# HueCodes/sudoku-vision

Hardware: AMD Instinct MI355X
Metric: end-to-end frames/sec (1080p->81 digits) (higher is better)
Workload: dtype f32

## Files before the change

### include/sudoku_vision_hip.h

```cpp
#ifndef SUDOKU_VISION_HIP_H
#define SUDOKU_VISION_HIP_H

#include <stddef.h>
#include <stdint.h>

#ifdef __cplusplus
extern "C" {
#endif

typedef struct sv_ctx sv_ctx;

typedef enum sv_status {
    SV_OK = 0,
    SV_ERR_BAD_ARG = -1,
    SV_ERR_HIP = -2,
    SV_ERR_NO_WEIGHTS = -3,
    SV_ERR_UNSUPPORTED = -4,
    SV_ERR_DEGENERATE = -5,
    SV_ERR_BUFFER = -6
} sv_status;

#define SV_CNN_PARAMS 421642
#define SV_CELLS 81
#define SV_CELL_PX 784
// ... 23 lines not shown

int sv_conv_kernel_info(sv_ctx *ctx, int *algo, int *mfma_f32_conv2_per_cell, int *mfma_f32_conv1_per_cell,
                        int *mfma_f16_conv_per_cell, int *mfma_f16_fc_per_cell);

int sv_load_weights_f32(sv_ctx *ctx, const float *blob);


int sv_gray_u8(sv_ctx *ctx, const uint8_t *bgr , int n, int H, int W, ptrdiff_t pitch,
               ptrdiff_t img_stride, uint8_t *gray , void *stream);

int sv_blur_u8(sv_ctx *ctx, const uint8_t *src , int n, int H, int W, int ksize,
               uint8_t *dst , void *stream);

int sv_adaptive_threshold_u8(sv_ctx *ctx, const uint8_t *src , int n, int H, int W,
                             int block, double c, int type_inv, uint8_t *dst , void *stream);

int sv_preprocess_u8(sv_ctx *ctx, const uint8_t *bgr , int n, int H, int W, ptrdiff_t pitch,
                     ptrdiff_t img_stride, uint8_t *binary , void *stream);

int sv_preprocess_warp_cells_u8(sv_ctx *ctx, const uint8_t *bgr , int n, int H, int W, ptrdiff_t pitch, ptrdiff_t img_stride,
                                uint8_t *binary , const double *minv , uint8_t *cells , void *stream);

int sv_preprocess_bits_u8(sv_ctx *ctx, const uint8_t *bgr , int n, int H, int W, ptrdiff_t pitch,
                          ptrdiff_t img_stride, uint32_t *bits , void *stream);

int sv_despeckle_bits(sv_ctx *ctx, uint32_t *bits , int n, int H, int W, void *stream);

int sv_despeckle_u8(sv_ctx *ctx, const uint8_t *binary , int n, int H, int W,
                    uint8_t *out , uint32_t *packed , void *stream);

long sv_sparse_bits_record_bytes(int H, int W, long cap_values);
int sv_pack_sparse_bits(sv_ctx *ctx, const uint32_t *bits , int n, int H, int W,
                        uint8_t *records , long record_stride, void *stream);

int sv_copy_to_pinned_host(sv_ctx *ctx, const void *src , void *dst_host , size_t bytes, void *stream);


int sv_find_grid_corners_u8(const uint8_t *binary , int H, int W, ptrdiff_t pitch,
                            double min_area_ratio, double epsilon_ratio, int *corners );

int sv_find_grid_corners_batch_u8(const uint8_t *binary , int n, int H, int W, ptrdiff_t pitch,
                                  ptrdiff_t img_stride, double min_area_ratio, double epsilon_ratio,
                                  int *corners , uint8_t *found , int threads);

int sv_find_grid_corners_bits_batch(const uint32_t *bits , int n, int H, int W,
                                    double min_area_ratio, double epsilon_ratio,
                                    int *corners , uint8_t *found , int threads);

int sv_host_pool_set_affinity(const int *cpus , int n);

int sv_find_grid_corners_sparse_batch(const uint8_t *records , long record_stride, int n, int H, int W,
                                      double min_area_ratio, double epsilon_ratio,
                                      int *corners , uint8_t *found , int threads);

int sv_sparse_bits_expand(const uint8_t *record , int H, int W, uint32_t *bits );

int sv_find_contours_u8(const uint8_t *binary , int H, int W, ptrdiff_t pitch,
                        int *points , long cap_points, int *sizes ,
                        int cap_contours, long *n_points, int *n_contours);

int sv_find_contours_bits(const uint32_t *bits , int H, int W, int *points, long cap_points, int *sizes, int cap_contours,
                          long *n_points, int *n_contours);

int sv_contour_area_i32(const int *xy , int n, double *area);
int sv_arc_length_i32(const int *xy , int n, int closed, double *length);
int sv_approx_poly_dp_i32(const int *xy , int n, double epsilon, int closed,
// ... 157 lines not shown
```

### sudoku-vision_amd/_native.py

```python
import ctypes as C
import os

_HERE = os.path.dirname(os.path.abspath(__file__))
LIB_PATH = os.path.join(_HERE, "csrc", "libsudokuvision_hip.so")
XCHECK_LIB_PATH = os.path.join(_HERE, "csrc", "libsudokuvision_xcheck.so")
ABI_VERSION = 2

SV_OK = 0
ERR_NAMES = {-1: "SV_ERR_BAD_ARG", -2: "SV_ERR_HIP", -3: "SV_ERR_NO_WEIGHTS", -4: "SV_ERR_UNSUPPORTED",
             -5: "SV_ERR_DEGENERATE", -6: "SV_ERR_BUFFER"}

_p, _i, _l, _d, _f, _pd = C.c_void_p, C.c_int, C.c_long, C.c_double, C.c_float, C.c_ssize_t

SIGNATURES = {
    "sv_version": [],
    "sv_last_error": [],
    "sv_ctx_create": [_i, C.POINTER(_p)],
    "sv_ctx_destroy": [_p],
    "sv_ctx_reserve": [_p, _l],
    "sv_ctx_set_precision": [_p, _i],
    "sv_load_weights_f32": [_p, _p],
    "sv_timing_begin": [_p],
    "sv_timing_end": [_p, _p, _p, _i],
    "sv_ctx_set_cnn_kernels": [_p, _i],
    "sv_conv_kernel_info": [_p, _p, _p, _p, _p, _p],
    "sv_gray_u8": [_p, _p, _i, _i, _i, _pd, _pd, _p, _p],
    "sv_blur_u8": [_p, _p, _i, _i, _i, _i, _p, _p],
    "sv_adaptive_threshold_u8": [_p, _p, _i, _i, _i, _i, _d, _i, _p, _p],
    "sv_preprocess_u8": [_p, _p, _i, _i, _i, _pd, _pd, _p, _p],
    "sv_solve_sudoku": [_p, _p, _p],
    "sv_despeckle_u8": [_p, _p, _i, _i, _i, _p, _p, _p],
    "sv_preprocess_bits_u8": [_p, _p, _i, _i, _i, _pd, _pd, _p, _p],
    "sv_preprocess_warp_cells_u8": [_p, _p, _i, _i, _i, _pd, _pd, _p, _p, _p, _p],
    "sv_despeckle_bits": [_p, _p, _i, _i, _i, _p],
    "sv_copy_to_pinned_host": [_p, _p, _p, C.c_size_t, _p],
    "sv_sparse_bits_record_bytes": [_i, _i, _l],
    "sv_pack_sparse_bits": [_p, _p, _i, _i, _i, _p, _l, _p],
    "sv_find_grid_corners_sparse_batch": [_p, _l, _i, _i, _i, _d, _d, _p, _p, _i],
    "sv_sparse_bits_expand": [_p, _i, _i, _p],
    "sv_host_pool_set_affinity": [_p, _i],
    "sv_find_grid_corners_bits_batch": [_p, _i, _i, _i, _d, _d, _p, _p, _i],
    "sv_corners_to_minv": [_p, _i, _i, _f, _p],
    "sv_corners_to_minv_batch": [_p, _i, _i, _f, _p, _p],
    "sv_find_grid_corners_u8": [_p, _i, _i, _pd, _d, _d, _p],
    "sv_find_grid_corners_batch_u8": [_p, _i, _i, _i, _pd, _pd, _d, _d, _p, _p, _i],
    "sv_find_contours_u8": [_p, _i, _i, _pd, _p, _l, _p, _i, _p, _p],
    "sv_find_contours_bits": [_p, _i, _i, _p, _l, _p, _i, _p, _p],
    "sv_contour_area_i32": [_p, _i, _p],
    "sv_arc_length_i32": [_p, _i, _i, _p],
    "sv_approx_poly_dp_i32": [_p, _i, _d, _i, _p, _p],
    "sv_warp_perspective_u8": [_p, _p, _i, _i, _pd, _i, _p, _i, _p, _p],
    "sv_extract_cells_u8": [_p, _p, _i, _i, _pd, _i, _i, _i, _i, _p, _p],
    "sv_warp_cells_u8": [_p, _p, _i, _i, _i, _pd, _pd, _p, _p, _p],
    "sv_resize_linear_u8": [_p, _p, _i, _i, _pd, _p, _i, _i, _p],
    "sv_cell_ink_ratio_u8": [_p, _p, _l, _i, _p, _p, _p],
    "sv_preprocess_cells_u8": [_p, _p, _l, _p, _p],
    "sv_jpeg_parse": [_p, C.c_size_t, _p],
    "sv_jpeg_entropy_decode": [_p, C.c_size_t, _p, _p, _i],
    "sv_jpeg_entropy_decode_sparse": [_p, C.c_size_t, _p, _p, _p, _l, _p, _p, _i],
    "sv_jpeg_entropy_decode_batch": [_p, _p, _i, _p, _p, _p, _p, _p, _p, _p, _i, _p],
    "sv_jpeg_reconstruct_bgr_u8": [_p, _p, _p, _p, _p, _pd, _p],
    "sv_jpeg_reconstruct_sparse_bgr_u8": [_p, _p, _p, _p, _p, _p, _p, _pd, _p],
    "sv_softmax_topk_f32": [_p, _p, _l, _i, _p, _p, _p],
    "sv_cnn_forward_f32": [_p, _p, _l, _p, _p, _p, _p],
    "sv_cnn_forward_cells_u8": [_p, _p, _l, _i, _p, _p, _p, _p],
    "sv_frames_to_digits": [_p, _p, _i, _i, _i, _pd, _pd, _p, _i, _p, _p, _p, _p, _p],
    "sv_load_weights_v3_f32": [_p, _p, _l, _i],
    "sv_cnn3_forward_f32": [_p, _p, _l, _p, _p, _p, _p, _p],
    "sv_cnn3_forward_cells_u8": [_p, _p, _l, _i, _p, _p, _p, _p],
    "sv_frames_to_digits_v3": [_p, _p, _i, _i, _i, _pd, _pd, _p, _i, _p, _p, _p, _p, _p],
# ... 73 lines not shown
```

### sudoku-vision_amd/csrc/k4_despeckle.hip

```cpp
#include "sv_device.h"
#include "sv_internal.h"

namespace {

typedef unsigned long long u64;
typedef unsigned int u32;

__device__ __forceinline__ u64 lane_shift_up(u64 v)
{
    const u32 lo = (u32)__builtin_amdgcn_update_dpp(0, (int)(u32)v, 0x138, 0xf, 0xf, true);
    const u32 hi = (u32)__builtin_amdgcn_update_dpp(0, (int)(u32)(v >> 32), 0x138, 0xf, 0xf, true);
    return ((u64)hi << 32) | lo;
}
__device__ __forceinline__ u64 lane_shift_down(u64 v)
{
    const u32 lo = (u32)__builtin_amdgcn_update_dpp(0, (int)(u32)v, 0x130, 0xf, 0xf, true);
    const u32 hi = (u32)__builtin_amdgcn_update_dpp(0, (int)(u32)(v >> 32), 0x130, 0xf, 0xf, true);
    return ((u64)hi << 32) | lo;
}
__device__ __forceinline__ u64 fill_runs(u64 f, u64 fr, u64 g)
{
    u64 up = ((f + g) ^ f) & f;
    const u64 gr = __brevll(g | up);
    const u64 dn = ((fr + gr) ^ fr) & fr;
// ... 145 lines not shown
        if (ok1[t] && (u32)(keep >> 32) != (u32)(f[t] >> 32)) row[k0[t] + 1] = (u32)(keep >> 32);
    }
}

__global__ __launch_bounds__(512) void k_despeckle_bits_band(u32 *__restrict__ bits, int H, int wpr, int pitch, int ox, int oy, int tiles_x, int tiles_y)
{
    extern __shared__ u32 band[];
    const int lane = threadIdx.x & 63, wave = threadIdx.x >> 6;
    const int ty = blockIdx.x % tiles_y;
    const long frame = blockIdx.x / tiles_y;
    const int y0 = ty * T - oy;
    u32 *img = bits + frame * H * (long)wpr;
    for (int r = wave; r < T; r += 8) {
        const int y = y0 + r;
        const bool ok = y >= 0 && y < H;
        for (int k = lane; k < wpr; k += 64) band[r * pitch + k] = ok ? img[(long)y * wpr + k] : 0u;
    }
    __syncthreads();
    const int y = y0 + lane;
    const bool row_ok = y >= 0 && y < H;
    u32 *row = img + (long)(row_ok ? y : 0) * wpr;
    const u32 *brow = band + lane * pitch;
    for (int tx = wave; tx < tiles_x; tx += 8) {
        const int k0 = (tx * T - ox) >> 5;
        const bool ok0 = k0 >= 0 && k0 < wpr, ok1 = k0 + 1 < wpr;
        const u64 f = (ok0 ? (u64)brow[k0] : 0ull) | (ok1 ? (u64)brow[k0 + 1] << 32 : 0ull);
        const u64 keep = ring_connected(f, lane);
        if (keep == f || !row_ok) continue;
        if (ok0 && (u32)keep != (u32)f) row[k0] = (u32)keep;
        if (ok1 && (u32)(keep >> 32) != (u32)(f >> 32)) row[k0 + 1] = (u32)(keep >> 32);
    }
}

__global__ __launch_bounds__(256) void k_copy_to_host(const uint4 *__restrict__ src, uint4 *__restrict__ dst, size_t n16, const u8 *__restrict__ tail_src,
                                                      u8 *__restrict__ tail_dst, int tail)
{
    for (size_t i = blockIdx.x * (size_t)256 + threadIdx.x; i < n16; i += (size_t)gridDim.x * 256) dst[i] = src[i];
    if (blockIdx.x == 0 && (int)threadIdx.x < tail) tail_dst[threadIdx.x] = tail_src[threadIdx.x];
}

template <bool KEEP>
__global__ __launch_bounds__(1024) void k_pack_sparse(const u32 *__restrict__ bits, int H, int wpr, int gpr, u8 *__restrict__ records, long stride,
                                                      unsigned cap_values)
{
    extern __shared__ u32 cnt[];
    const int tid = threadIdx.x, lane = tid & 63, wave = tid >> 6, G = H * gpr;
    u32 *wsum = cnt + G;
    const u32 *fb = bits + (size_t)blockIdx.x * H * wpr;
    u8 *rec = records + (size_t)blockIdx.x * stride;
    u64 *masks = (u64 *)(rec + 8);
    u32 *values = (u32 *)(rec + 8 + 8 * (size_t)G);
    constexpr int U = 8, TRIPS = 9;
    u32 kept[KEEP ? TRIPS : 1][U];
    auto load_trip = [&](int g0, u32 (&w)[U]) {
#pragma unroll
        for (int u = 0; u < U; u++) {
            const int g = g0 + u, y = g / gpr, k = (g - y * gpr) * 64 + lane;
            w[u] = (g < G && k < wpr) ? fb[(size_t)y * wpr + k] : 0u;
        }
    };
    auto count_trip = [&](int g0, const u32 (&w)[U]) {
#pragma unroll
        for (int u = 0; u < U; u++) {
            const u64 m = __ballot(w[u] != 0);
            if (lane == 0 && g0 + u < G) { masks[g0 + u] = m; cnt[g0 + u] = (u32)__popcll(m); }
        }
// ... 53 lines not shown
}

int svk_despeckle_bits(uint32_t *bits, int n, int H, int W, hipStream_t s)
{
    for (int pass = 0; pass < 2; pass++) {
        const int o = pass ? T / 2 : 0;
        const int tiles_x = (W + o + T - 1) / T, tiles_y = (H + o + T - 1) / T;
        const int wpr = W >> 5, pitch = wpr | 1;
        if ((size_t)T * pitch * 4 <= 65536) {
            hipLaunchKernelGGL(k_despeckle_bits_band, dim3((unsigned)(n * tiles_y)), dim3(512), (size_t)T * pitch * 4, s, bits, H, wpr, pitch, o, o, tiles_x, tiles_y);
            SV_LAUNCH_CHECK("k_despeckle_bits_band");
            continue;
        }
        const long ngroups = (long)n * ((tiles_x + TPW - 1) / TPW) * tiles_y;
        hipLaunchKernelGGL(k_despeckle_bits, dim3((unsigned)((ngroups + 3) / 4)), dim3(256), 0, s, bits, H, wpr, o, o, tiles_x, tiles_y, ngroups);
        SV_LAUNCH_CHECK("k_despeckle_bits");
    }
    return SV_OK;
}

int svk_pack_sparse_bits(const u32 *bits, int n, int H, int W, u8 *records, long stride, hipStream_t s)
{
    const int wpr = W >> 5, gpr = (wpr + 63) / 64, G = H * gpr;
    const long cap = (stride - 8 - 8L * G) / 4;
    const unsigned capu = (unsigned)(cap > 0xffffffffL ? 0xffffffffL : cap);
    if (G <= 16 * 9 * 8)
        hipLaunchKernelGGL(k_pack_sparse<true>, dim3((unsigned)n), dim3(1024), (size_t)(G + 16) * 4, s, bits, H, wpr, gpr, records, stride, capu);
    else
        hipLaunchKernelGGL(k_pack_sparse<false>, dim3((unsigned)n), dim3(1024), (size_t)(G + 16) * 4, s, bits, H, wpr, gpr, records, stride, capu);
    SV_LAUNCH_CHECK("k_pack_sparse");
    return SV_OK;
}

int svk_copy_to_host(const void *src, void *dst_host, size_t bytes, hipStream_t s)
{
    const size_t n16 = bytes / 16;
    const int tail = (int)(bytes - n16 * 16);
    size_t wgs = (n16 + 255) / 256;
    wgs = wgs < 1 ? 1 : (wgs > 64 ? 64 : wgs);
    hipLaunchKernelGGL(k_copy_to_host, dim3((unsigned)wgs), dim3(256), 0, s, (const uint4 *)src, (uint4 *)dst_host, n16, (const u8 *)src + n16 * 16,
                       (u8 *)dst_host + n16 * 16, tail);
    SV_LAUNCH_CHECK("k_copy_to_host");
    return SV_OK;
}

int svk_despeckle(const u8 *src, int n, int H, int W, u8 *dst, u32 *packed, hipStream_t s)
{
    for (int pass = 0; pass < 2; pass++) {
        const int o = pass ? T / 2 : 0;
        const int tiles_x = (W + o + T - 1) / T, tiles_y = (H + o + T - 1) / T;
        const long ntiles = (long)n * tiles_x * tiles_y;
        hipLaunchKernelGGL(k_despeckle, dim3((unsigned)((ntiles + 3) / 4)), dim3(256), 0, s, pass ? dst : src, dst, pass ? packed : (u32 *)nullptr, H, W, o, o,
                           tiles_x, tiles_y, ntiles);
        SV_LAUNCH_CHECK("k_despeckle");
    }
    return SV_OK;
}
```

### sudoku-vision_amd/csrc/sv_api.cpp

```cpp
#include <algorithm>
#include <cmath>
#include <cstdlib>
#include <cstring>
#include <vector>

#include "sv_internal.h"

static thread_local char g_err[512] = "";

int sv_fail(int code, const char *fmt, ...)
{
    va_list ap;
    va_start(ap, fmt);
    vsnprintf(g_err, sizeof g_err, fmt, ap);
    va_end(ap);
    return code;
}

extern "C" const char *sv_last_error(void) { return g_err; }
extern "C" int sv_version(void) { return 2; }

extern "C" int sv_ctx_create(int device, sv_ctx **out)
{
    if (!out) return sv_fail(SV_ERR_BAD_ARG, "sv_ctx_create: out is NULL");
    int count = 0;
    SV_HIP(hipGetDeviceCount(&count));
    if (device < 0 || device >= count) return sv_fail(SV_ERR_BAD_ARG, "sv_ctx_create: device %d of %d", device, count);
    SV_HIP(hipSetDevice(device));
    hipDeviceProp_t prop;
    SV_HIP(hipGetDeviceProperties(&prop, device));
    sv_ctx *c = new sv_ctx();
    c->device = device;
    c->num_cus = prop.multiProcessorCount > 0 ? prop.multiProcessorCount : 256;
    *out = c;
    return SV_OK;
}

template <class W>
static void free_weights(W &w)
{
    for (void *p : w.allocs) (void)hipFree(p);
    w = W();
}

extern "C" int sv_ctx_destroy(sv_ctx *ctx)
{
    if (!ctx) return SV_OK;
    (void)hipSetDevice(ctx->device);
    free_weights(ctx->w);
    free_weights(ctx->w3);
    if (ctx->v3_act) (void)hipFree(ctx->v3_act);
    if (ctx->features) (void)hipFree(ctx->features);
    if (ctx->cells) (void)hipFree(ctx->cells);
    if (ctx->cells2) (void)hipFree(ctx->cells2);
    if (ctx->jpeg_planes) (void)hipFree(ctx->jpeg_planes);
    if (ctx->pp2) (void)hipFree(ctx->pp2);
    if (ctx->k1_list) (void)hipFree(ctx->k1_list);
    if (ctx->range_flag) (void)hipFree(ctx->range_flag);
    for (auto &t : ctx->timeline) { (void)hipEventDestroy(t.t0); (void)hipEventDestroy(t.t1); }
    for (auto &e : ctx->event_pool) (void)hipEventDestroy(e);
    delete ctx;
    return SV_OK;
}

int sv_ensure_scratch(sv_ctx *ctx, long cells)
{
    if (cells <= ctx->cap_cells) return SV_OK;
    SV_HIP(hipSetDevice(ctx->device));
    if (ctx->features) SV_HIP(hipFree(ctx->features));
    if (ctx->cells) SV_HIP(hipFree(ctx->cells));
    if (ctx->cells2) SV_HIP(hipFree(ctx->cells2));
    ctx->features = nullptr;
    ctx->cells = nullptr;
    ctx->cells2 = nullptr;
    ctx->cap_cells = 0;
    SV_HIP(hipMalloc((void **)&ctx->features, sizeof(float) * 3136 * (size_t)cells));
    SV_HIP(hipMalloc((void **)&ctx->cells, (size_t)SV_CELL_PX * (size_t)cells));
    SV_HIP(hipMalloc((void **)&ctx->cells2, (size_t)SV_CELL_PX * (size_t)cells));
    ctx->cap_cells = cells;
    return SV_OK;
}

static int sv_ensure_scratch_v3(sv_ctx *ctx, long cells)
{
    const long want = cells < SV_V3_SUBBATCH ? cells : SV_V3_SUBBATCH;
    if (want <= ctx->cap_v3) return SV_OK;
    SV_HIP(hipSetDevice(ctx->device));
    if (ctx->v3_act) SV_HIP(hipFree(ctx->v3_act));
    ctx->v3_act = nullptr;
// ... 314 lines not shown

extern "C" int sv_despeckle_bits(sv_ctx *ctx, uint32_t *bits, int n, int H, int W, void *stream)
{
    REQUIRE(ctx && bits, "NULL argument");
    REQUIRE(n > 0 && H > 0 && W > 0 && W % 32 == 0, "bad shape (W must be a multiple of 32)");
    return svk_despeckle_bits(bits, n, H, W, S(stream));
}

extern "C" int sv_despeckle_u8(sv_ctx *ctx, const uint8_t *binary, int n, int H, int W, uint8_t *out, uint32_t *packed, void *stream)
{
    REQUIRE(ctx && binary && out, "NULL argument");
    REQUIRE(n > 0 && H > 0 && W > 0, "bad shape");
    REQUIRE(!packed || W % 32 == 0, "packed output needs W % 32 == 0");
    return svk_despeckle(binary, n, H, W, out, packed, S(stream));
}

extern "C" long sv_sparse_bits_record_bytes(int H, int W, long cap_values)
{
    if (H <= 0 || W <= 0 || (W & 31) || cap_values < 0) return -1;
    const long gpr = ((W >> 5) + 63) / 64;
    return (8 + 8 * gpr * H + 4 * cap_values + 15) / 16 * 16;
}

extern "C" int sv_pack_sparse_bits(sv_ctx *ctx, const uint32_t *bits, int n, int H, int W, uint8_t *records, long record_stride, void *stream)
{
    REQUIRE(ctx && bits && records, "NULL argument");
    REQUIRE(n > 0 && H > 0 && W > 0 && W % 32 == 0, "bad shape (W must be a multiple of 32)");
    const long G = (long)H * (((W >> 5) + 63) / 64);
    REQUIRE(G <= 16000, "frame too large for the sparse record (more than 16000 row groups)");
    REQUIRE(record_stride % 8 == 0 && record_stride >= 8 + 8 * G + 4 && ((uintptr_t)records & 7) == 0, "record stride must be a multiple of 8 with room for the masks");
    return svk_pack_sparse_bits(bits, n, H, W, records, record_stride, S(stream));
}

extern "C" int sv_copy_to_pinned_host(sv_ctx *ctx, const void *src, void *dst_host, size_t bytes, void *stream)
{
    REQUIRE(ctx && src && dst_host, "NULL argument");
    REQUIRE((((uintptr_t)src | (uintptr_t)dst_host) & 15) == 0, "source and destination must be 16-byte aligned");
    if (bytes == 0) return SV_OK;
    hipPointerAttribute_t attr;
    if (hipPointerGetAttributes(&attr, dst_host) != hipSuccess || attr.type != hipMemoryTypeHost) {
        (void)hipGetLastError();
        return sv_fail(SV_ERR_BAD_ARG, "sv_copy_to_pinned_host: destination is not pinned (hipHostMalloc / hipHostRegister) host memory");
    }
    return svk_copy_to_host(src, dst_host, bytes, S(stream));
}

extern "C" int sv_warp_perspective_u8(sv_ctx *ctx, const uint8_t *img, int H, int W, ptrdiff_t pitch, int channels, const double *minv, int out_size, uint8_t *dst, void *stream)
{
    REQUIRE(ctx && img && minv && dst, "NULL argument");
    REQUIRE(H > 0 && W > 0 && out_size > 0 && out_size < 32768, "bad shape");
    REQUIRE(channels == 1 || channels == 3, "channels must be 1 or 3");
    REQUIRE(pitch >= (ptrdiff_t)W * channels, "pitch < row bytes");
    return svk_warp_perspective(img, H, W, pitch, channels, minv, out_size, dst, S(stream));
}

extern "C" int sv_extract_cells_u8(sv_ctx *ctx, const uint8_t *grid, int h, int w, ptrdiff_t pitch, int channels, int cell_size, int margin_h, int margin_w, uint8_t *cells, void *stream)
{
    REQUIRE(ctx && grid && cells, "NULL argument");
    REQUIRE(h >= 9 && w >= 9 && cell_size > 0, "bad shape");
    REQUIRE(channels == 1 || channels == 3, "channels must be 1 or 3");
    REQUIRE(margin_h >= 0 && margin_w >= 0 && h / 9 - 2 * margin_h > 0 && w / 9 - 2 * margin_w > 0, "margin leaves an empty cell");
    return svk_extract_cells(grid, h, w, pitch, channels, cell_size, margin_h, margin_w, cells, S(stream));
}

extern "C" int sv_warp_cells_u8(sv_ctx *ctx, const uint8_t *frames, int n, int H, int W, ptrdiff_t pitch, ptrdiff_t frame_stride, const double *minv, uint8_t *cells, void *stream)
{
// ... 258 lines not shown
```

### sudoku-vision_amd/csrc/sv_internal.h

```cpp
#pragma once
#include <hip/hip_runtime.h>
#include <cstdarg>
#include <cstdint>
#include <cstdio>
#include <vector>

#include "../../include/sudoku_vision_hip.h"
#ifdef SV_XCHECK
#include "../../include/sudoku_vision_xcheck.h"
#endif

typedef uint8_t u8;

struct sv_weights {
    float *conv1_w = nullptr;
    float *conv1_b = nullptr;
    float *conv2_wreg = nullptr;
    float *conv2_wino = nullptr;
    float *conv2_b = nullptr;
    float *fc1_wreg = nullptr;
    float *fc1_b = nullptr;
    unsigned short *conv2_wsplit = nullptr;
    unsigned short *conv2_bf16 = nullptr;
    unsigned short *fc1_bf16 = nullptr;
// ... 6 lines not shown
    bool h2_in_range = true;
    float h2_x_lo = 0.f, h2_x_hi = 0.f;
    float *fc2_w = nullptr;
    float *fc2_b = nullptr;
    bool loaded = false;
    std::vector<void *> allocs;
};

struct sv_conv3 { float *w = nullptr, *b = nullptr; };
struct sv_weights3 {
    sv_conv3 stem, conv1[5], conv2[5], shortcut[5];
    float *se1[5] = {}, *se2[5] = {};
    float *fc_w = nullptr, *fc_b = nullptr;
    float temperature = 1.f;
    bool use_se = true, loaded = false;
    std::vector<void *> allocs;
};

struct sv_ctx {
    int device = 0;
    int num_cus = 256;
    sv_weights w;
    sv_weights3 w3;
    float *v3_act = nullptr;
    long cap_v3 = 0;
    float *features = nullptr;
    u8 *cells = nullptr;
    u8 *cells2 = nullptr;
    long cap_cells = 0;
    u8 *jpeg_planes = nullptr;
    size_t cap_jpeg = 0;
    u8 *pp2 = nullptr;
    size_t cap_pp2 = 0;
    void *k1_list = nullptr;
    int precision = 0;
    int cnn_kernels = 0;
    int *range_flag = nullptr;
    bool x_fc_frame = false;
    int dev_ablate = 0;
    bool timing = false;
    struct timed { int kernel; hipEvent_t t0, t1; };
    std::vector<timed> timeline;
    std::vector<hipEvent_t> event_pool;
};

enum sv_kernel_id { SVK_PREPROCESS = 0, SVK_WARP_CELLS = 1, SVK_CONV_FEATURES = 2, SVK_FC_HEAD = 3, SVK_FUSED12 = 4, SVK_COUNT = 5 };

struct sv_time_scope {
    sv_ctx *ctx; hipStream_t s; int idx = -1;
    sv_time_scope(sv_ctx *c, int kernel, hipStream_t st);
    ~sv_time_scope();
};

int sv_fail(int code, const char *fmt, ...);

#define SV_HIP(expr)                                                                         \
    do {                                                                                     \
        hipError_t e_ = (expr);                                                              \
        if (e_ != hipSuccess) return sv_fail(SV_ERR_HIP, "%s: %s", #expr, hipGetErrorString(e_)); \
    } while (0)

#define SV_LAUNCH_CHECK(name)                                                                \
    do {                                                                                     \
        hipError_t e_ = hipGetLastError();                                                   \
        if (e_ != hipSuccess) return sv_fail(SV_ERR_HIP, "launch %s: %s", name, hipGetErrorString(e_)); \
    } while (0)
// ... 8 lines not shown
    SV_HIP(hipMemcpy(*dst, src, n * sizeof(T), hipMemcpyHostToDevice));
    return SV_OK;
}

enum sv_cnn_algo { SV_ALGO_F32MFMA = 0, SV_ALGO_X_WINOGRAD = 2, SV_ALGO_X_WSPLIT = 3, SV_ALGO_F16PAIR = 4 };

int svk_gray(const u8 *bgr, int n, int H, int W, ptrdiff_t pitch, ptrdiff_t img_stride, u8 *gray, hipStream_t s);
int svk_blur(const u8 *src, int n, int H, int W, int ksize, u8 *dst, hipStream_t s);
int svk_adaptive_threshold(const u8 *src, int n, int H, int W, int block, const float *taps, int idelta, int type_inv,
                           u8 *dst, hipStream_t s);
int svk_preprocess(sv_ctx *ctx, const u8 *bgr, int n, int H, int W, ptrdiff_t pitch, ptrdiff_t img_stride, u8 *binary, hipStream_t s);
int svk_preprocess_bits(sv_ctx *ctx, const u8 *bgr, int n, int H, int W, ptrdiff_t pitch, ptrdiff_t img_stride, uint32_t *bits, hipStream_t s);
int svk_despeckle_bits(uint32_t *bits, int n, int H, int W, hipStream_t s);
int svk_preprocess_mm_stats(sv_ctx *ctx, unsigned *ambiguous, unsigned long *capacity);
int svk_preprocess_mm_enable_stats(sv_ctx *ctx);
bool svk_preprocess_mm_supported(const u8 *bgr, int H, int W, ptrdiff_t pitch, ptrdiff_t img_stride, const void *out, bool bits);
int svk_preprocess_mm(sv_ctx *ctx, const u8 *bgr, int n, int H, int W, ptrdiff_t pitch, ptrdiff_t img_stride, u8 *out, bool bits, float *mean_dbg, hipStream_t s);
int svk_preprocess_warp_fused(sv_ctx *ctx, const u8 *bgr, int n, int H, int W, ptrdiff_t pitch, ptrdiff_t img_stride, u8 *binary, const double *minv, u8 *cells,
                              hipStream_t s);
int svk_warp_perspective(const u8 *img, int H, int W, ptrdiff_t pitch, int channels, const double *minv, int out_size,
                         u8 *dst, hipStream_t s);
int svk_extract_cells(const u8 *grid, int h, int w, ptrdiff_t pitch, int channels, int cell_size, int margin_h,
                      int margin_w, u8 *cells, hipStream_t s);
int svk_warp_cells(sv_ctx *ctx, const u8 *frames, int n, int H, int W, ptrdiff_t pitch, ptrdiff_t frame_stride, const double *minv,
                   u8 *cells, hipStream_t s);
int svk_cnn_forward(sv_ctx *ctx, const void *x, bool x_is_u8, int glue, long B, float *logits, u8 *digits, float *conf,
                    hipStream_t s);
int svk_pack_weights_f32mfma(sv_weights &w, const float *c2w, const float *f1w);
int svk_pack_weights_bf16(sv_weights &w, const float *c2w, const float *f1w);
int svk_pack_weights_h2(sv_weights &w, const float *c1w, const float *c1b, const float *c2w, const float *c2b, const float *f1w);

int svk_despeckle(const u8 *src, int n, int H, int W, u8 *dst, unsigned *packed, hipStream_t s);
int svk_pack_sparse_bits(const uint32_t *bits, int n, int H, int W, u8 *records, long stride, hipStream_t s);
int svk_copy_to_host(const void *src, void *dst_host, size_t bytes, hipStream_t s);
int svk_resize_linear(const u8 *src, int sh, int sw, ptrdiff_t pitch, u8 *dst, int dh, int dw, hipStream_t s);
int svk_cnn_forward_bf16(sv_ctx *ctx, const u8 *cells, long B, float *logits, u8 *digits, float *conf, hipStream_t s);
int svk_cnn_forward_h2(sv_ctx *ctx, const void *x, bool x_is_u8, long B, float *logits, u8 *digits, float *conf, const int *run_if_clear, hipStream_t s);
int svk_cell_ink_ratio(const u8 *cells, long B, int npx, float *ratio, int *otsu, hipStream_t s);
int svk_preprocess_cells(const u8 *cells, long B, u8 *out, hipStream_t s);
int svk_jpeg_reconstruct(sv_ctx *ctx, const sv_jpeg_info *info, const int16_t *coef, const uint64_t *masks, const uint32_t *offsets, const int16_t *values,
                         const uint16_t *quant, u8 *bgr, ptrdiff_t pitch, hipStream_t s);
int svk_softmax_topk(const float *logits, long B, int k, u8 *index, float *prob, hipStream_t s);
int svk_frame_quality_stats(const u8 *img, int n, int H, int W, ptrdiff_t pitch, ptrdiff_t img_stride, int C, long long *lap_sum, long long *lap_sqsum,
                            uint32_t *hist, hipStream_t s);
int svk_grid_line_coverage(const void *src, bool bits, int n, int H, int W, ptrdiff_t pitch, ptrdiff_t img_stride, const double *minv, uint32_t *counts,
                           hipStream_t s);
int svk_morphology(sv_ctx *ctx, const u8 *src, int n, int H, int W, ptrdiff_t pitch, ptrdiff_t img_stride, int op, int shape, int k, u8 *dst, hipStream_t s);
int svk_box_mean(const u8 *src, int n, int H, int W, ptrdiff_t pitch, ptrdiff_t img_stride, int k, u8 *dst, hipStream_t s);
int svk_threshold_sauvola(const u8 *src, int n, int H, int W, ptrdiff_t pitch, ptrdiff_t img_stride, int window, double k, u8 *dst, hipStream_t s);
int svk_gaussian_blur21(const u8 *src, int n, int H, int W, ptrdiff_t pitch, ptrdiff_t img_stride, u8 *dst, hipStream_t s);
int svk_clahe(sv_ctx *ctx, const u8 *src, int n, int H, int W, ptrdiff_t pitch, ptrdiff_t img_stride, double clip, int tiles_x, int tiles_y, u8 *dst, hipStream_t s);
int svk_divide_normalize(const u8 *gray, int n, int H, int W, ptrdiff_t pitch, ptrdiff_t img_stride, const u8 *background, u8 *dst, hipStream_t s);
int svk_threshold_count(const u8 *src, int n, int H, int W, ptrdiff_t pitch, ptrdiff_t img_stride, int thresh, int type_inv, u8 *dst, uint32_t *counts, hipStream_t s);
int svk_shadow_mask(const u8 *gray, int n, int H, int W, ptrdiff_t pitch, ptrdiff_t img_stride, const u8 *local_mean, int delta, u8 *mask, uint32_t *counts, hipStream_t s);
int svk_count_nonzero(const u8 *src, int n, int H, int W, ptrdiff_t pitch, ptrdiff_t img_stride, uint32_t *counts, hipStream_t s);

int svk_pack_weights_v3(sv_weights3 &w, const float *blob, bool use_se);
long svk_v3_blob_floats(bool use_se);
size_t svk_v3_scratch_bytes(long cells);
int svk_cnn3_forward(sv_ctx *ctx, const void *x, bool x_is_u8, long B, float *logits, float *features, u8 *digits, float *conf, hipStream_t s);

void sv_gaussian_taps_f32(int n, float *out);
```

### sudoku-vision_amd/pipeline.py

```python
import os
import time
from concurrent.futures import ThreadPoolExecutor
from dataclasses import dataclass, field

import numpy as np
import torch

from . import host
from .runtime import Context


def host_cpu_budget():
    n = len(os.sched_getaffinity(0)) if hasattr(os, "sched_getaffinity") else (os.cpu_count() or 1)
    for path, parse in (("/sys/fs/cgroup/cpu.max", lambda t: t.split()),
                        ("/sys/fs/cgroup/cpu/cpu.cfs_quota_us", lambda t: [t.strip(), open("/sys/fs/cgroup/cpu/cpu.cfs_period_us").read().strip()])):
        try:
            quota, period = parse(open(path).read())
            if quota not in ("max", "-1"):
                n = min(n, max(1, int(quota) // int(period)))
            break
        except (OSError, ValueError):
            continue
    return n


def _parse_cpulist(text):
    cpus = set()
    for part in text.strip().split(","):
        if part:
            lo, _, hi = part.partition("-")
            cpus.update(range(int(lo), int(hi or lo) + 1))
    return cpus


def gpu_local_cpus(device):
    try:
        p = torch.cuda.get_device_properties(device)
        path = f"/sys/bus/pci/devices/{p.pci_domain_id:04x}:{p.pci_bus_id:02x}:{p.pci_device_id:02x}.0/local_cpulist"
        cpus = _parse_cpulist(open(path).read())
    except (OSError, ValueError, AttributeError, RuntimeError):
        return None
    if hasattr(os, "sched_getaffinity"):
        cpus &= os.sched_getaffinity(0)
    return cpus or None


class FramePipeline:
    def __init__(self, ctx: Context, H: int, W: int, chunk: int = 32, host_threads=None, min_area_ratio=0.1, glue=0, despeckle=True, sparse=True, depth=5, cpu_affinity="auto", bits_direct=True,
                 quality=False):
        self.ctx, self.H, self.W, self.chunk = ctx, H, W, chunk
        self.depth = depth = max(2, int(depth))
        self.host_threads = host_threads or max(1, host_cpu_budget() - 2)
        self.min_area_ratio = min_area_ratio
        self.despeckle = bool(despeckle) and min_area_ratio * H * W > 61 * 61
        self.glue = glue
        dev = ctx.device
        self.s_pre = torch.cuda.Stream(dev)
        self.s_d2h = torch.cuda.Stream(dev)
        self.s_cls = torch.cuda.Stream(dev)
        self.packed = self.despeckle and W % 32 == 0
        self.bits_direct = bool(bits_direct)
        self.sparse = self.packed and bool(sparse) and H * ((W // 32 + 63) // 64) <= 16000
        if self.packed:
            self.dev_bits = [torch.empty((chunk, H, W // 32), dtype=torch.int32, device=dev) for _ in range(depth)]
        if self.sparse:
            cap = H * (W // 32) // 3 if sparse is True else int(sparse)
            self.rec_bytes = host.sparse_bits_record_bytes(H, W, cap)
            self.pinned = [torch.empty((chunk, self.rec_bytes), dtype=torch.uint8).pin_memory() for _ in range(depth)]
            self.dev_rec = [torch.empty((chunk, self.rec_bytes), dtype=torch.uint8, device=dev) for _ in range(depth)]
            self.s_side = torch.cuda.Stream(dev)
        elif self.packed:
            self.pinned = [torch.empty((chunk, H, W // 32), dtype=torch.int32).pin_memory() for _ in range(depth)]
        else:
            self.pinned = [torch.empty((chunk, H, W), dtype=torch.uint8).pin_memory() for _ in range(depth)]
        self.dev_bin = None
        self.minv_pin = [torch.empty((chunk, 9), dtype=torch.float64).pin_memory() for _ in range(depth)]
        self.minv_dev = [torch.empty((chunk, 9), dtype=torch.float64, device=dev) for _ in range(depth)]
        self.cpus = gpu_local_cpus(dev) if cpu_affinity == "auto" else (set(cpu_affinity) if cpu_affinity else None)
        if self.cpus:
            host.set_pool_affinity(self.cpus)
        self.pool = ThreadPoolExecutor(1, initializer=(lambda: os.sched_setaffinity(0, self.cpus)) if self.cpus and hasattr(os, "sched_setaffinity") else None)
        self.dense_fallbacks = 0
        self.quality = bool(quality)
        if self.quality:
            self.q_bin = [None] * depth
        ctx.reserve(chunk * 81)

    def _search(self, slot, m, ev):
        ev.synchronize()
        if self.sparse:
            corners, found = host.find_grid_corners_sparse_batch(self.pinned[slot][:m].numpy(), self.H, self.W, self.min_area_ratio, 0.02, self.host_threads)
            over = np.nonzero(found == 2)[0]
            if over.size:
                with torch.cuda.stream(self.s_side):
                    dense = self.dev_bits[slot][torch.from_numpy(over).to(self.ctx.device)].cpu().numpy()
# ... 49 lines not shown
            q_cnt = torch.zeros((n, 20), dtype=torch.int32, device=dev)
        if total is None:
            starts = [(s0, min(self.chunk, n - s0)) for _ in range(repeat) for s0 in range(0, n, self.chunk)]
        else:
            starts = [((k * self.chunk) % n, min(self.chunk, total - k * self.chunk)) for k in range((total + self.chunk - 1) // self.chunk)]
        pending = []
        free_ev = [None] * self.depth

        def classify(item):
            fut, slot, s, m = item
            corners, found = fut.result()
            corners_all[s:s + m], found_all[s:s + m] = corners, found
            with torch.cuda.stream(self.s_cls):
                self.minv_dev[slot][:m].copy_(self.minv_pin[slot][:m], non_blocking=True)
                sub = {k: out[k][s:s + m] for k in ("logits", "digits", "conf")}
                self.ctx.frames_to_digits(frames[s:s + m], self.minv_dev[slot][:m], out=sub, glue=self.glue)
                if self.quality:
                    self.ctx.grid_line_coverage(self.q_bin[slot][:m], self.minv_dev[slot][:m], out=q_cnt[s:s + m])
                if not found.all():
                    out["digits"][s:s + m][torch.from_numpy(~found).to(dev)] = 0
                ev = torch.cuda.Event(blocking=True)
                ev.record(self.s_cls)
                free_ev[slot] = ev

        for i, (s, m) in enumerate(starts):
            slot = i % self.depth
            if free_ev[slot] is not None:
                free_ev[slot].synchronize()
            with torch.cuda.stream(self.s_pre):
                if bits_direct:
                    b = self.ctx.preprocess_bits(frames[s:s + m], out=self.dev_bits[slot][:m])
                    if self.quality:
                        self.q_bin[slot][:m].copy_(b)
                    b = self.ctx.despeckle_bits(b)
                else:
                    b = self.ctx.preprocess(frames[s:s + m], out=self.dev_bin[slot][:m])
                    if self.quality:
                        self.q_bin[slot][:m].copy_(b)
                if self.packed:
                    if not bits_direct:
                        b = self.ctx.despeckle(b, out=b, packed=self.dev_bits[slot][:m])
                    if self.sparse:
                        b = self.ctx.pack_sparse_bits(b, self.dev_rec[slot])
                elif self.despeckle:
                    b = self.ctx.despeckle(b, out=b)
                ready = torch.cuda.Event()
                ready.record(self.s_pre)
                if self.quality:
                    self.ctx.frame_quality_stats(frames[s:s + m], out=(q_s1[s:s + m], q_s2[s:s + m], q_hist[s:s + m]))
            with torch.cuda.stream(self.s_d2h):
                self.s_d2h.wait_event(ready)
                self.pinned[slot][:m].copy_(b, non_blocking=True)
                ev = torch.cuda.Event(blocking=True)
                ev.record(self.s_d2h)
            pending.append((self.pool.submit(self._search, slot, m, ev), slot, s, m))
            if len(pending) > self.depth - 2:
                classify(pending.pop(0))
        while pending:
            classify(pending.pop(0))
        cur.wait_stream(self.s_cls)
        out["corners"], out["found"] = corners_all, found_all
        if self.quality:
            from .cv.grid_quality import scores_from_stats
            cur.wait_stream(self.s_pre)
            s1, s2, hist, cnt = (t.cpu().numpy() for t in (q_s1, q_s2, q_hist, q_cnt))
            out["quality"] = scores_from_stats(s1, s2, hist, cnt, corners_all, found_all, self.H * self.W).astype(np.float32)
        return out


def recognize_image(image, model_state_dict=None, ctx=None, glue=Context.GLUE_RUNPY, top_k=0, quality=False, preprocess="v1", model="v1"):
    from .runtime import default_context
    if preprocess not in ("v1", "v2"):
        raise ValueError(f"preprocess must be 'v1' or 'v2', got {preprocess!r}")
    if model not in ("v1", "v3"):
        raise ValueError(f"model must be 'v1' or 'v3', got {model!r}")
# ... 177 lines not shown
```

### sudoku-vision_amd/runtime.py

```python
import ctypes as C
import threading

import numpy as np
import torch

from . import _native

_V1_LAYOUT = (("conv1.weight", (32, 1, 3, 3)), ("conv1.bias", (32,)), ("conv2.weight", (64, 32, 3, 3)), ("conv2.bias", (64,)),
              ("fc1.weight", (128, 3136)), ("fc1.bias", (128,)), ("fc2.weight", (10, 128)), ("fc2.bias", (10,)))


_V3_BLOCKS = ((32, 32, 1), (32, 64, 2), (64, 64, 1), (64, 128, 2), (128, 128, 1))


def v3_layout(use_se=True):
    def bn(prefix, c):
        return [(f"{prefix}.{n}", (c,)) for n in ("weight", "bias", "running_mean", "running_var")]
    out = [("temperature", (1,)), ("stem.0.weight", (32, 1, 3, 3))] + bn("stem.1", 32)
    for i, (cin, c, stride) in enumerate(_V3_BLOCKS, 1):
        L = f"layer{i}"
        out += [(f"{L}.conv1.weight", (c, cin, 3, 3))] + bn(f"{L}.bn1", c) + [(f"{L}.conv2.weight", (c, c, 3, 3))] + bn(f"{L}.bn2", c)
        if use_se:
            out += [(f"{L}.se.excite.0.weight", (c // 4, c)), (f"{L}.se.excite.2.weight", (c, c // 4))]
        if stride != 1 or cin != c:
# ... 251 lines not shown
    def preprocess_bits(self, frames, out=None):
        frames, pitch, fstride = _frame_layout(frames, self.device)
        n, H, W = frames.shape[0], frames.shape[1], frames.shape[2]
        if W % 32:
            raise ValueError("preprocess_bits needs W % 32 == 0")
        out = self._out(out, (n, H, W // 32), torch.int32, "out")
        self._check(self._lib.sv_preprocess_bits_u8(self._h, _ptr(frames), n, H, W, pitch, fstride, _ptr(out), _stream_ptr()), "sv_preprocess_bits_u8")
        return out

    def despeckle_bits(self, bits):
        self._out(_dev_tensor(bits, "bits", torch.int32, self.device, ndim=3), bits.shape, torch.int32, "bits")
        n, H, wpr = bits.shape
        self._check(self._lib.sv_despeckle_bits(self._h, _ptr(bits), n, H, wpr * 32, _stream_ptr()), "sv_despeckle_bits")
        return bits

    def despeckle(self, binary, out=None, packed=None):
        binary = _dev_tensor(binary, "binary", torch.uint8, self.device, ndim=3).contiguous()
        n, H, W = binary.shape
        out = self._out(out, (n, H, W), torch.uint8, "out")
        if packed is not None:
            self._out(packed, (n, H, W // 32), torch.int32, "packed")
        self._check(self._lib.sv_despeckle_u8(self._h, _ptr(binary), n, H, W, _ptr(out), _opt_ptr(packed),
                                                    _stream_ptr()), "sv_despeckle_u8")
        return out if packed is None else packed

    def pack_sparse_bits(self, bits, records):
        _dev_tensor(bits, "bits", torch.int32, self.device, ndim=3)
        _dev_tensor(records, "records", torch.uint8, self.device, ndim=2)
        n, H, wpr = bits.shape
        if records.shape[0] < n or not records.is_contiguous() or not bits.is_contiguous():
            raise TypeError("records must be a contiguous uint8 [>=n, stride] device tensor")
        self._check(self._lib.sv_pack_sparse_bits(self._h, _ptr(bits), n, H, wpr * 32, _ptr(records), records.shape[1], _stream_ptr()),
                      "sv_pack_sparse_bits")
        return records[:n]

    def copy_to_pinned(self, src, dst):
        _dev_tensor(src, "src", None, self.device)
        if not dst.is_pinned() or not dst.is_contiguous() or not src.is_contiguous():
            raise TypeError("copy_to_pinned needs a contiguous device tensor and a contiguous pinned host tensor")
        nbytes = src.numel() * src.element_size()
        if nbytes != dst.numel() * dst.element_size():
            raise ValueError("size mismatch")
        self._check(self._lib.sv_copy_to_pinned_host(self._h, _ptr(src), _ptr(dst), nbytes, _stream_ptr()), "sv_copy_to_pinned_host")
        return dst

    @staticmethod
    def corners_to_minv(corners, output_size=450, inset_ratio=0.0):
        c = np.ascontiguousarray(np.asarray(corners, dtype=np.float32).reshape(-1, 8))
        out = np.empty((c.shape[0], 3, 3), np.float64)
        _native.check(_native.lib().sv_corners_to_minv(c.ctypes.data_as(C.c_void_p), c.shape[0], int(output_size), float(inset_ratio),
                                                       out.ctypes.data_as(C.c_void_p)), "sv_corners_to_minv")
        return out

    @staticmethod
    def corners_to_minv_batch(corners, output_size=450, inset_ratio=0.0):
        c = np.ascontiguousarray(np.asarray(corners, dtype=np.float32).reshape(-1, 8))
        out = np.empty((c.shape[0], 3, 3), np.float64)
        ok = np.empty(c.shape[0], np.uint8)
        _native.check(_native.lib().sv_corners_to_minv_batch(c.ctypes.data_as(C.c_void_p), c.shape[0], int(output_size), float(inset_ratio),
                                                             out.ctypes.data_as(C.c_void_p), ok.ctypes.data_as(C.c_void_p)), "sv_corners_to_minv_batch")
        return out, ok.astype(bool)

    def minv_to_device(self, minv):
        return torch.from_numpy(np.ascontiguousarray(minv, np.float64)).to(self.device)

    def warp_perspective(self, img, minv_dev, output_size):
# ... 305 lines not shown
```

Measured before the change: 193,600.

## Fuse second despeckle pass with sparse bit packing via decoupled lookback

Adds a kernel that runs the second (offset-tile) despeckle pass and then packs the surviving bit rows into the sparse record in the same block. Per-band word counts are combined across bands with a decoupled-lookback prefix through a tagged global state buffer. This removes the separate pack kernel launch and its re-read of the bit planes. The cost is spin-waiting between blocks and an extra state allocation on the context, and the pipeline enables it by default.

After: 184,500. -4.7%, worse.

```diff
diff --git a/include/sudoku_vision_hip.h b/include/sudoku_vision_hip.h
--- a/include/sudoku_vision_hip.h
+++ b/include/sudoku_vision_hip.h
@@ -79,6 +79,9 @@
 long sv_sparse_bits_record_bytes(int H, int W, long cap_values);
 int sv_pack_sparse_bits(sv_ctx *ctx, const uint32_t *bits , int n, int H, int W,
                         uint8_t *records , long record_stride, void *stream);
+
+int sv_despeckle_pack_bits(sv_ctx *ctx, uint32_t *bits , int n, int H, int W,
+                           uint8_t *records , long record_stride, void *stream);
 
 int sv_copy_to_pinned_host(sv_ctx *ctx, const void *src , void *dst_host , size_t bytes, void *stream);
 
diff --git a/sudoku-vision_amd/_native.py b/sudoku-vision_amd/_native.py
--- a/sudoku-vision_amd/_native.py
+++ b/sudoku-vision_amd/_native.py
@@ -36,6 +36,7 @@
     "sv_copy_to_pinned_host": [_p, _p, _p, C.c_size_t, _p],
     "sv_sparse_bits_record_bytes": [_i, _i, _l],
     "sv_pack_sparse_bits": [_p, _p, _i, _i, _i, _p, _l, _p],
+    "sv_despeckle_pack_bits": [_p, _p, _i, _i, _i, _p, _l, _p],
     "sv_find_grid_corners_sparse_batch": [_p, _l, _i, _i, _i, _d, _d, _p, _p, _i],
     "sv_sparse_bits_expand": [_p, _i, _i, _p],
     "sv_host_pool_set_affinity": [_p, _i],
diff --git a/sudoku-vision_amd/csrc/k4_despeckle.hip b/sudoku-vision_amd/csrc/k4_despeckle.hip
--- a/sudoku-vision_amd/csrc/k4_despeckle.hip
+++ b/sudoku-vision_amd/csrc/k4_despeckle.hip
@@ -201,6 +201,95 @@
     }
 }
 
+__global__ __launch_bounds__(512) void k_despeckle_bits_band_pack(u32 *__restrict__ bits, int H, int wpr, int pitch, int tiles_x, int tiles_y, int gpr,
+                                                                   u8 *__restrict__ records, long stride, unsigned cap_values, u64 *__restrict__ state, u32 tag)
+{
+    extern __shared__ u32 band[];
+    const int lane = threadIdx.x & 63, wave = threadIdx.x >> 6, tid = threadIdx.x;
+    const int n = gridDim.x / tiles_y;
+    const int ty = blockIdx.x / n;
+    const int frame = blockIdx.x % n;
+    const int slot = frame * tiles_y + ty;
+    const int y0 = ty * T - T / 2;
+    u32 *img = bits + (long)frame * H * wpr;
+    u32 *cnt = band + T * pitch;
+    for (int r = wave; r < T; r += 8) {
+        const int y = y0 + r;
+        const bool ok = y >= 0 && y < H;
+        for (int k = lane; k < wpr; k += 64) band[r * pitch + k] = ok ? img[(long)y * wpr + k] : 0u;
+    }
+    __syncthreads();
+    {
+        const int y = y0 + lane;
+        const bool row_ok = y >= 0 && y < H;
+        u32 *row = img + (long)(row_ok ? y : 0) * wpr;
+        u32 *brow = band + lane * pitch;
+        for (int tx = wave; tx < tiles_x; tx += 8) {
+            const int k0 = (tx * T - T / 2) >> 5;
+            const bool ok0 = k0 >= 0 && k0 < wpr, ok1 = k0 + 1 < wpr;
+            const u64 f = (ok0 ? (u64)brow[k0] : 0ull) | (ok1 ? (u64)brow[k0 + 1] << 32 : 0ull);
+            const u64 keep = ring_connected(f, lane);
+            if (keep == f || !row_ok) continue;
+            if (ok0 && (u32)keep != (u32)f) row[k0] = brow[k0] = (u32)keep;
+            if (ok1 && (u32)(keep >> 32) != (u32)(f >> 32)) row[k0 + 1] = brow[k0 + 1] = (u32)(keep >> 32);
+        }
+    }
+    __syncthreads();
+    const int r_lo = y0 < 0 ? -y0 : 0, r_hi = H - y0 < T ? H - y0 : T, ng = (r_hi - r_lo) * gpr;
+    const int G = H * gpr;
+    u8 *rec = records + (size_t)frame * stride;
+    u64 *masks = (u64 *)(rec + 8) + (size_t)(y0 + r_lo) * gpr;
+    u32 *values = (u32 *)(rec + 8 + 8 * (size_t)G);
+#pragma unroll
+    for (int u = 0; u < T / 8; u++) {
+        const int r = r_lo + wave + 8 * u;
+        if (r >= r_hi) break;
+        for (int g = 0; g < gpr; g++) {
+            const int j = (r - r_lo) * gpr + g, k = g * 64 + lane;
+            const u64 m = __ballot(k < wpr && band[r * pitch + k] != 0);
+            if (lane == 0) { masks[j] = m; cnt[j] = (u32)__popcll(m); }
+        }
+    }
+    __syncthreads();
+    u32 *off = cnt + T * gpr;
+    u32 total = 0;
+    for (int c = 0; c < ng; c += 64) {
+        const u32 v = c + lane < ng ? cnt[c + lane] : 0u;
+        u32 incl = v;
+#pragma unroll
+        for (int d = 1; d < 64; d <<= 1) {
+            const u32 t = __shfl_up(incl, d);
+            if (lane >= d) incl += t;
+        }
+        if (c + lane < ng) off[c + lane] = total + incl - v;
+        total += __shfl(incl, 63);
+    }
+    if (tid == 0) __hip_atomic_store(state + slot, ((u64)tag << 32) | total, __ATOMIC_RELAXED, __HIP_MEMORY_SCOPE_AGENT);
+    u32 base = 0;
+    for (int i = lane; i < ty; i += 64) {
+        u64 x;
+        while (((x = __hip_atomic_load(state + slot - ty + i, __ATOMIC_RELAXED, __HIP_MEMORY_SCOPE_AGENT)) >> 32) != tag) __builtin_amdgcn_s_sleep(2);
+        base += (u32)x;
+    }
+#pragma unroll
+    for (int d = 32; d; d >>= 1) base += __shfl_xor(base, d);
+#pragma unroll
+    for (int u = 0; u < T / 8; u++) {
+        const int r = r_lo + wave + 8 * u;
+        if (r >= r_hi) break;
+        for (int g = 0; g < gpr; g++) {
+            const int j = (r - r_lo) * gpr + g, k = g * 64 + lane;
+            const u32 w = k < wpr ? band[r * pitch + k] : 0u;
+            const u64 m = __ballot(w != 0);
+            if (w) {
+                const u32 pos = base + off[j] + (u32)__popcll(m & ((1ull << lane) - 1));
+                if (pos < cap_values) values[pos] = w;
+            }
+        }
+    }
+    if (ty == tiles_y - 1 && tid == 0) { ((u32 *)rec)[0] = base + total; ((u32 *)rec)[1] = cap_values; }
+}
+
 __global__ __launch_bounds__(256) void k_copy_to_host(const uint4 *__restrict__ src, uint4 *__restrict__ dst, size_t n16, const u8 *__restrict__ tail_src,
                                                       u8 *__restrict__ tail_dst, int tail)
 {
@@ -320,6 +409,40 @@
     return SV_OK;
 }
 
+constexpr int SLOT_SETS = 8;
+int svk_despeckle_pack_bits(sv_ctx *ctx, uint32_t *bits, int n, int H, int W, u8 *records, long stride, hipStream_t s)
+{
+    const int wpr = W >> 5, pitch = wpr | 1, gpr = (wpr + 63) / 64, G = H * gpr;
+    const size_t lds = ((size_t)T * pitch + 2 * (size_t)T * gpr) * 4;
+    if (lds > 65536) {
+        const int rc = svk_despeckle_bits(bits, n, H, W, s);
+        return rc ? rc : svk_pack_sparse_bits(bits, n, H, W, records, stride, s);
+    }
+    const int o = T / 2, tiles_y = (H + o + T - 1) / T;
+    const long slots = (long)n * tiles_y;
+    if (slots > ctx->cap_pack_slots) {
+        SV_HIP(hipSetDevice(ctx->device));
+        if (ctx->pack_slots) SV_HIP(hipFree(ctx->pack_slots));
+        ctx->pack_slots = nullptr;
+        ctx->cap_pack_slots = 0;
+        SV_HIP(hipMalloc((void **)&ctx->pack_slots, sizeof(u64) * SLOT_SETS * (size_t)slots));
+        SV_HIP(hipMemset(ctx->pack_slots, 0, sizeof(u64) * SLOT_SETS * (size_t)slots));
+        ctx->cap_pack_slots = slots;
+    }
+    if (++ctx->pack_calls == 0) ctx->pack_calls = SLOT_SETS;
+    const u32 tag = ctx->pack_calls;
+    u64 *state = (u64 *)ctx->pack_slots + (size_t)(tag % SLOT_SETS) * ctx->cap_pack_slots;
+    const long cap = (stride - 8 - 8L * G) / 4;
+    const unsigned capu = (unsigned)(cap > 0xffffffffL ? 0xffffffffL : cap);
+    hipLaunchKernelGGL(k_despeckle_bits_band, dim3((unsigned)(n * (long)((H + T - 1) / T))), dim3(512), (size_t)T * pitch * 4, s, bits, H, wpr, pitch, 0, 0, (W + T - 1) / T,
+                       (H + T - 1) / T);
+    SV_LAUNCH_CHECK("k_despeckle_bits_band");
+    hipLaunchKernelGGL(k_despeckle_bits_band_pack, dim3((unsigned)slots), dim3(512), lds, s, bits, H, wpr, pitch, (W + o + T - 1) / T, tiles_y, gpr, records, stride, capu,
+                       state, tag);
+    SV_LAUNCH_CHECK("k_despeckle_bits_band_pack");
+    return SV_OK;
+}
+
 int svk_copy_to_host(const void *src, void *dst_host, size_t bytes, hipStream_t s)
 {
     const size_t n16 = bytes / 16;
diff --git a/sudoku-vision_amd/csrc/sv_api.cpp b/sudoku-vision_amd/csrc/sv_api.cpp
--- a/sudoku-vision_amd/csrc/sv_api.cpp
+++ b/sudoku-vision_amd/csrc/sv_api.cpp
@@ -55,6 +55,7 @@
     if (ctx->cells2) (void)hipFree(ctx->cells2);
     if (ctx->jpeg_planes) (void)hipFree(ctx->jpeg_planes);
     if (ctx->pp2) (void)hipFree(ctx->pp2);
+    if (ctx->pack_slots) (void)hipFree(ctx->pack_slots);
     if (ctx->k1_list) (void)hipFree(ctx->k1_list);
     if (ctx->range_flag) (void)hipFree(ctx->range_flag);
     for (auto &t : ctx->timeline) { (void)hipEventDestroy(t.t0); (void)hipEventDestroy(t.t1); }
@@ -435,6 +436,16 @@
     return svk_pack_sparse_bits(bits, n, H, W, records, record_stride, S(stream));
 }
 
+extern "C" int sv_despeckle_pack_bits(sv_ctx *ctx, uint32_t *bits, int n, int H, int W, uint8_t *records, long record_stride, void *stream)
+{
+    REQUIRE(ctx && bits && records, "NULL argument");
+    REQUIRE(n > 0 && H > 0 && W > 0 && W % 32 == 0, "bad shape (W must be a multiple of 32)");
+    const long G = (long)H * (((W >> 5) + 63) / 64);
+    REQUIRE(G <= 16000, "frame too large for the sparse record (more than 16000 row groups)");
+    REQUIRE(record_stride % 8 == 0 && record_stride >= 8 + 8 * G + 4 && ((uintptr_t)records & 7) == 0, "record stride must be a multiple of 8 with room for the masks");
+    return svk_despeckle_pack_bits(ctx, bits, n, H, W, records, record_stride, S(stream));
+}
+
 extern "C" int sv_copy_to_pinned_host(sv_ctx *ctx, const void *src, void *dst_host, size_t bytes, void *stream)
 {
     REQUIRE(ctx && src && dst_host, "NULL argument");
diff --git a/sudoku-vision_amd/csrc/sv_internal.h b/sudoku-vision_amd/csrc/sv_internal.h
--- a/sudoku-vision_amd/csrc/sv_internal.h
+++ b/sudoku-vision_amd/csrc/sv_internal.h
@@ -62,6 +62,9 @@
     size_t cap_jpeg = 0;
     u8 *pp2 = nullptr;
     size_t cap_pp2 = 0;
+    void *pack_slots = nullptr;
+    long cap_pack_slots = 0;
+    unsigned pack_calls = 0;
     void *k1_list = nullptr;
     int precision = 0;
     int cnn_kernels = 0;
@@ -136,6 +139,7 @@
 
 int svk_despeckle(const u8 *src, int n, int H, int W, u8 *dst, unsigned *packed, hipStream_t s);
 int svk_pack_sparse_bits(const uint32_t *bits, int n, int H, int W, u8 *records, long stride, hipStream_t s);
+int svk_despeckle_pack_bits(sv_ctx *ctx, uint32_t *bits, int n, int H, int W, u8 *records, long stride, hipStream_t s);
 int svk_copy_to_host(const void *src, void *dst_host, size_t bytes, hipStream_t s);
 int svk_resize_linear(const u8 *src, int sh, int sw, ptrdiff_t pitch, u8 *dst, int dh, int dw, hipStream_t s);
 int svk_cnn_forward_bf16(sv_ctx *ctx, const u8 *cells, long B, float *logits, u8 *digits, float *conf, hipStream_t s);
diff --git a/sudoku-vision_amd/pipeline.py b/sudoku-vision_amd/pipeline.py
--- a/sudoku-vision_amd/pipeline.py
+++ b/sudoku-vision_amd/pipeline.py
@@ -47,7 +47,7 @@
 
 class FramePipeline:
     def __init__(self, ctx: Context, H: int, W: int, chunk: int = 32, host_threads=None, min_area_ratio=0.1, glue=0, despeckle=True, sparse=True, depth=5, cpu_affinity="auto", bits_direct=True,
-                 quality=False):
+                 quality=False, fused_pack=True):
         self.ctx, self.H, self.W, self.chunk = ctx, H, W, chunk
         self.depth = depth = max(2, int(depth))
         self.host_threads = host_threads or max(1, host_cpu_budget() - 2)
@@ -61,6 +61,7 @@
         self.packed = self.despeckle and W % 32 == 0
         self.bits_direct = bool(bits_direct)
         self.sparse = self.packed and bool(sparse) and H * ((W // 32 + 63) // 64) <= 16000
+        self.fused_pack = bool(fused_pack)
         if self.packed:
             self.dev_bits = [torch.empty((chunk, H, W // 32), dtype=torch.int32, device=dev) for _ in range(depth)]
         if self.sparse:
@@ -176,7 +177,8 @@
                     b = self.ctx.preprocess_bits(frames[s:s + m], out=self.dev_bits[slot][:m])
                     if self.quality:
                         self.q_bin[slot][:m].copy_(b)
-                    b = self.ctx.despeckle_bits(b)
+                    fused = self.sparse and self.fused_pack
+                    b = self.ctx.despeckle_pack_bits(b, self.dev_rec[slot]) if fused else self.ctx.despeckle_bits(b)
                 else:
                     b = self.ctx.preprocess(frames[s:s + m], out=self.dev_bin[slot][:m])
                     if self.quality:
@@ -184,7 +186,7 @@
                 if self.packed:
                     if not bits_direct:
                         b = self.ctx.despeckle(b, out=b, packed=self.dev_bits[slot][:m])
-                    if self.sparse:
+                    if self.sparse and not (bits_direct and self.fused_pack):
                         b = self.ctx.pack_sparse_bits(b, self.dev_rec[slot])
                 elif self.despeckle:
                     b = self.ctx.despeckle(b, out=b)
diff --git a/sudoku-vision_amd/runtime.py b/sudoku-vision_amd/runtime.py
--- a/sudoku-vision_amd/runtime.py
+++ b/sudoku-vision_amd/runtime.py
@@ -307,6 +307,16 @@
             raise TypeError("records must be a contiguous uint8 [>=n, stride] device tensor")
         self._check(self._lib.sv_pack_sparse_bits(self._h, _ptr(bits), n, H, wpr * 32, _ptr(records), records.shape[1], _stream_ptr()),
                       "sv_pack_sparse_bits")
+        return records[:n]
+
+    def despeckle_pack_bits(self, bits, records):
+        self._out(_dev_tensor(bits, "bits", torch.int32, self.device, ndim=3), bits.shape, torch.int32, "bits")
+        _dev_tensor(records, "records", torch.uint8, self.device, ndim=2)
+        n, H, wpr = bits.shape
+        if records.shape[0] < n or not records.is_contiguous():
+            raise TypeError("records must be a contiguous uint8 [>=n, stride] device tensor")
+        self._check(self._lib.sv_despeckle_pack_bits(self._h, _ptr(bits), n, H, wpr * 32, _ptr(records), records.shape[1], _stream_ptr()),
+                      "sv_despeckle_pack_bits")
         return records[:n]
 
     def copy_to_pinned(self, src, dst):
```
